# siyi-wind/MDViT

Hardware: AMD Instinct MI355X
Metric: 512x512 images/sec MDViT train step (fwd+bwd, two-sweep, AdamW) (higher is better)
Workload: dtype bf16x3 (fp32 storage; GEMM operands split hi+lo bf16, fp32 accumulate); 1 GPU; MDViT Sup+MLPFM train step, 4 domain(s) x bs=4 per GPU, 512x512, drop_rate=0.1 drop_path=0.1, bf16x3 GEMMs, data-parallel x1

## Files before the change

### include/mdvit_hip.h

```cpp
#ifndef MDVIT_HIP_H
#define MDVIT_HIP_H

#include <stddef.h>
#include <stdint.h>

#ifdef __cplusplus
extern "C" {
#endif

#define MDVIT_ABI_VERSION 1

enum {
    MDVIT_OK = 0,
    MDVIT_E_SHAPE = 1,
    MDVIT_E_DTYPE = 2,
    MDVIT_E_ALIGN = 3,
    MDVIT_E_WORKSPACE = 4,
    MDVIT_E_HIP = 5
};

enum { MDVIT_EPI_NONE = 0, MDVIT_EPI_GELU_DUAL = 1, MDVIT_EPI_DGELU = 2 };
enum { MDVIT_ACT_NONE = 0, MDVIT_ACT_HSWISH = 1, MDVIT_ACT_RELU = 2 };

const char* mdvit_last_error(void);
// ... 124 lines not shown
int mdvit_mlp_rc_bwd(const float* gm, const float* x, const void* W1p, const float* b1, const void* W2tp, const void* W1tp, float* dx_parts, float* dW1, float* db1,
                     float* dW2, void* ws, size_t ws_bytes, int32_t M, int32_t C, int32_t hidden, float drop_p, uint32_t key1_0, uint32_t key1_1,
                     const uint32_t* drop_seed, int32_t accumulate, void* stream);
size_t mdvit_mlp_rc_wgrad_ws_bytes(int32_t M, int32_t C, int32_t hidden);
int mdvit_mlp_rc_dgrad_masked(const float* g, const float* x, const void* W1p, const float* b1, const void* W2tp, const void* W1tp, float* dx, int32_t M, int32_t C,
                              int32_t hidden, float drop_p, uint32_t key1_0, uint32_t key1_1, const uint32_t* drop_seed, float mask_drop_p, uint32_t mask_key0,
                              uint32_t mask_key1, const uint32_t* mask_seed, const float* rowscale, int32_t rows_per_scale, void* stream);
int mdvit_mlp_rc16_dgrad_masked(const float* g, const float* x, const void* W1p, const float* b1, const void* W2tp, const void* W1tp, float* du, float* dx, float* gm_out,
                                int32_t M, int32_t C, int32_t hidden, float drop_p, uint32_t key1_0, uint32_t key1_1, const uint32_t* drop_seed, float mask_drop_p,
                                uint32_t mask_key0, uint32_t mask_key1, const uint32_t* mask_seed, const float* rowscale, int32_t rows_per_scale, void* stream);
int mdvit_mlp_rc16_dgrad_masked_hbf16(const float* g, const float* x, const void* W1p, const float* b1, const void* W2tp, const void* W1tp, float* du, float* dx,
                                      float* gm_out, int32_t M, int32_t C, int32_t hidden, float drop_p, uint32_t key1_0, uint32_t key1_1, const uint32_t* drop_seed,
                                      float mask_drop_p, uint32_t mask_key0, uint32_t mask_key1, const uint32_t* mask_seed, const float* rowscale,
                                      int32_t rows_per_scale, void* stream);
int mdvit_mlp_rc_wgrad_masked(const float* g, const float* x, const void* W1p, const float* b1, const void* W2tp, float* dW1, float* db1, float* dW2, void* ws,
                              size_t ws_bytes, int32_t M, int32_t C, int32_t hidden, float drop_p, uint32_t key1_0, uint32_t key1_1, const uint32_t* drop_seed,
                              float mask_drop_p, uint32_t mask_key0, uint32_t mask_key1, const uint32_t* mask_seed, const float* rowscale, int32_t rows_per_scale,
                              int32_t accumulate, void* stream);
int mdvit_mlp_rc_bwd_masked(const float* g, const float* x, const void* W1p, const float* b1, const void* W2tp, const void* W1tp, float* dx_parts, float* dW1, float* db1,
                            float* dW2, void* ws, size_t ws_bytes, int32_t M, int32_t C, int32_t hidden, float drop_p, uint32_t key1_0, uint32_t key1_1,
                            const uint32_t* drop_seed, float mask_drop_p, uint32_t mask_key0, uint32_t mask_key1, const uint32_t* mask_seed, const float* rowscale,
                            int32_t rows_per_scale, int32_t accumulate, void* stream);
int mdvit_mlp_mask_config(int32_t fold);
int mdvit_gemm_ledger(int32_t enable);
int mdvit_gemm_ledger_read(int32_t index, char* name, int32_t cap, int64_t* launches, double* flop, double* bytes);
int mdvit_gemm_sampler(const char* symbol, int32_t stride);
int mdvit_gemm_sampler_read(int32_t index, char* name, int32_t cap, int64_t* seen, int64_t* timed, double* ms);
int mdvit_mlp_rc_config(int32_t fwd_variant);
int mdvit_mlp_rc_planes(int32_t planes);
int mdvit_block_config(int32_t mlp_bwd_fused);
int mdvit_mlp_rc_wgrad(const float* gm, const float* x, const void* W1p, const float* b1, const void* W2tp, float* dW1, float* db1, float* dW2,
                       void* ws, size_t ws_bytes, int32_t M, int32_t C, int32_t hidden, float drop_p, uint32_t key1_0, uint32_t key1_1,
                       const uint32_t* drop_seed, int32_t accumulate, void* stream);

typedef struct MdvitBlockDesc {
    int32_t B, H, W, C, heads, hidden, s3, s5, s7, ln_groups, D, da_hidden, precision;
    float eps, drop_p;
    uint32_t key_proj[2], key_fc1[2], key_fc2[2];
    const uint32_t* drop_seed;
    const float* rowscale1; const float* rowscale2;
    const float* label;
    const float *cpe_w, *cpe_b, *n1_g, *n1_b, *qkv_w, *qkv_b, *w3, *b3, *w5, *b5, *w7, *b7, *da_w1, *da_b1, *da_w2, *da_b2, *proj_w, *proj_b, *n2_g, *n2_b, *fc1_w, *fc1_b,
        *fc2_w, *fc2_b;
    const float *qkv_wt, *proj_wt, *fc1_wt, *fc2_wt;
    const void *fc1_p, *fc2_p, *fc2t_p, *fc1t_p;
    const void *qkv_p, *proj_p, *projt_p, *qkvt_p;
// ... 252 lines not shown
```

### mdvit_amd/_lib.py

```python
from __future__ import annotations

import ctypes as C
import os
import re
from typing import List

_HERE = os.path.dirname(os.path.abspath(__file__))
LIB_PATH = os.environ.get("MDVIT_HIP_LIB") or os.path.join(_HERE, "lib", "libmdvit_hip.so")
HEADER_PATH = os.path.join(_HERE, "..", "include", "mdvit_hip.h")

EPI_NONE, EPI_GELU_DUAL, EPI_DGELU = 0, 1, 2
ACT_NONE, ACT_HSWISH, ACT_RELU = 0, 1, 2

f32p = C.c_void_p
vp = C.c_void_p
i32 = C.c_int32
i64 = C.c_int64
u32 = C.c_uint32
f32 = C.c_float


class GemmDesc(C.Structure):
    _fields_ = [
        ("A", vp), ("B", vp), ("C", vp), ("C2", vp),
# ... 107 lines not shown
    "mdvit_block_config": [i32],
    "mdvit_gemm_ledger": [i32],
    "mdvit_gemm_ledger_read": [i32, C.c_char_p, i32, C.POINTER(i64), C.POINTER(C.c_double), C.POINTER(C.c_double)],
    "mdvit_gemm_sampler": [C.c_char_p, i32],
    "mdvit_gemm_sampler_read": [i32, C.c_char_p, i32, C.POINTER(i64), C.POINTER(i64), C.POINTER(C.c_double)],
    "mdvit_mlp_rc_fwd": [vp, vp, vp, vp, vp, vp, vp, i32, vp, i32, i32, i32, f32, u32, u32, u32, u32, vp, vp],
    "mdvit_linear_rc": [vp, i64, vp, i64, vp, vp, i64, i32, i32, i32, f32, u32, u32, vp, i32, vp, i64, vp, vp],
    "mdvit_linear_rc_ln": [vp, vp, vp, i32, f32, vp, vp, vp, vp, i64, vp, vp, i64, i32, i32, i32, vp],
    "mdvit_mlp_rc_fwd_ln": [vp, vp, vp, i32, f32, vp, vp, vp, vp, vp, vp, vp, vp, i32, vp, vp, i32, i32, i32, f32, u32, u32, u32, u32, vp, vp],
    "mdvit_mlp_rc16_fwd": [vp, vp, vp, vp, vp, vp, vp, i32, vp, vp, i32, i32, i32, f32, u32, u32, u32, u32, vp, vp],
    "mdvit_mlp_rc_dgrad": [vp, vp, vp, vp, vp, vp, vp, i32, i32, i32, f32, u32, u32, vp, vp],
    "mdvit_mlp_rc16_dgrad": [vp, vp, vp, vp, vp, vp, vp, vp, i32, i32, i32, f32, u32, u32, vp, vp],
    "mdvit_mlp_rc_fwd_ln_hbf16": [vp, vp, vp, i32, f32, vp, vp, vp, vp, vp, vp, vp, vp, i32, vp, vp, i32, i32, i32, f32, u32, u32, u32, u32, vp, vp],
    "mdvit_mlp_rc16_fwd_hbf16": [vp, vp, vp, vp, vp, vp, vp, i32, vp, vp, i32, i32, i32, f32, u32, u32, u32, u32, vp, vp],
    "mdvit_mlp_rc16_dgrad_hbf16": [vp, vp, vp, vp, vp, vp, vp, vp, i32, i32, i32, f32, u32, u32, vp, vp],
    "mdvit_mlp_rc_wgrad": [vp, vp, vp, vp, vp, vp, vp, vp, vp, C.c_size_t, i32, i32, i32, f32, u32, u32, vp, i32, vp],
    "mdvit_mlp_rc_bwd": [vp, vp, vp, vp, vp, vp, vp, vp, vp, vp, vp, C.c_size_t, i32, i32, i32, f32, u32, u32, vp, i32, vp],
    "mdvit_mlp_rc_dgrad_masked": [vp, vp, vp, vp, vp, vp, vp, i32, i32, i32, f32, u32, u32, vp, f32, u32, u32, vp, vp, i32, vp],
    "mdvit_mlp_rc16_dgrad_masked": [vp, vp, vp, vp, vp, vp, vp, vp, vp, i32, i32, i32, f32, u32, u32, vp, f32, u32, u32, vp, vp, i32, vp],
    "mdvit_mlp_rc16_dgrad_masked_hbf16": [vp, vp, vp, vp, vp, vp, vp, vp, vp, i32, i32, i32, f32, u32, u32, vp, f32, u32, u32, vp, vp, i32, vp],
    "mdvit_mlp_rc_wgrad_masked": [vp, vp, vp, vp, vp, vp, vp, vp, vp, C.c_size_t, i32, i32, i32, f32, u32, u32, vp, f32, u32, u32, vp, vp, i32, i32, vp],
    "mdvit_mlp_rc_bwd_masked": [vp, vp, vp, vp, vp, vp, vp, vp, vp, vp, vp, C.c_size_t, i32, i32, i32, f32, u32, u32, vp, f32, u32, u32, vp, vp, i32, i32, vp],
    "mdvit_mlp_mask_config": [i32],
    "mdvit_imgconv_fwd": [vp, vp, vp, i32, i32, i32, i32, i32, i32, vp],
    "mdvit_imgconv_wgrad": [vp, vp, vp, vp, C.c_size_t, i32, i32, i32, i32, i32, i32, i32, vp],
    "mdvit_maxpool3x3s2_fwd": [vp, vp, vp, i32, i32, i32, i32, vp],
    "mdvit_maxpool3x3s2_bwd": [vp, vp, vp, i32, i32, i32, i32, vp],
    "mdvit_resize_ac_fwd": [vp, vp, i32, i32, i32, i32, i32, i32, vp],
    "mdvit_resize_ac_bwd": [vp, vp, i32, i32, i32, i32, i32, i32, vp],
    "mdvit_ew": [vp, vp, vp, i64, i32, vp],
    "mdvit_add3": [vp, vp, vp, vp, i64, vp],
    "mdvit_add_parts": [vp, vp, C.POINTER(vp), i32, i64, vp, vp],
    "mdvit_add_bcast": [vp, vp, vp, i32, i64, vp],
    "mdvit_sum_batch": [vp, vp, i32, i64, vp],
    "mdvit_gate_fwd": [vp, vp, vp, i32, i64, i32, i32, vp],
    "mdvit_gate_bwd": [vp, vp, vp, vp, vp, vp, C.c_size_t, i32, i64, i32, i32, vp],
    "mdvit_imgconv_im2col": [vp, vp, i32, i32, i32, i32, i32, i32, vp],
    "mdvit_chanpool_fwd": [vp, vp, vp, i64, i32, vp],
    "mdvit_chanpool_bwd": [vp, vp, vp, i64, i32, vp],
    "mdvit_conv7x7_2to1_fwd": [vp, vp, vp, i32, i32, i32, vp],
    "mdvit_conv7x7_2to1_bwd": [vp, vp, vp, vp, vp, i32, i32, i32, vp],
    "mdvit_bn1_fwd": [vp, vp, vp, vp, vp, vp, vp, vp, i64, i32, i32, f32, f32, vp],
    "mdvit_bn1_bwd": [vp, vp, vp, vp, vp, vp, i64, i32, i32, vp],
    "mdvit_subsample2": [vp, vp, i32, i32, i32, i32, i32, vp],
    "mdvit_patchify": [vp, vp, i32, i32, i32, i32, i32, vp],
    "mdvit_dropout2d": [vp, vp, i32, i64, i32, f32, u32, u32, vp, vp],
# ... 204 lines not shown
```

### mdvit_amd/csrc/mlp_rc.hip

```cpp
#include "common.h"
#include <type_traits>
#ifndef RC_ABL
#define RC_ABL 0
#endif

typedef float rc_f32x16 __attribute__((ext_vector_type(16)));
typedef __bf16 rc_bf16x8 __attribute__((ext_vector_type(8)));
typedef unsigned rc_u4 __attribute__((ext_vector_type(4)));
typedef unsigned rc_u2 __attribute__((ext_vector_type(2)));
typedef float rc_f4 __attribute__((ext_vector_type(4)));
typedef short rc_v4i16 __attribute__((ext_vector_type(4)));
typedef short rc_v8i16 __attribute__((ext_vector_type(8)));
typedef __attribute__((address_space(3))) rc_v4i16* rc_lds_v4i16_ptr;

namespace {

template <int ROWB>
__device__ __forceinline__ int rc_swz(int row) {
    if (ROWB == 64) return (row >> 2) & 3;
    if (ROWB == 128) return (((row >> 1) & 1) << 2) | ((row >> 2) & 3);
    return row & 15;
}

template <int ROWB>
__device__ __forceinline__ void rc_glds_piece(const uint16_t* __restrict__ src, long ld, int piece, int lane, char* tile) {
    constexpr int LPR = ROWB / 16, RPP = 1024 / ROWB;
    const int row = piece * RPP + lane / LPR;
    const int lc = (lane % LPR) ^ rc_swz<ROWB>(row);
    __builtin_amdgcn_global_load_lds(src + (long)row * ld + (lc << 3), (__attribute__((address_space(3))) void*)(tile + piece * 1024), 16, 0, 0);
}

template <int ROWB>
__device__ __forceinline__ rc_bf16x8 rc_frag(const char* tile, int row, int chunk) {
    return __builtin_bit_cast(rc_bf16x8, *reinterpret_cast<const rc_u4*>(tile + row * ROWB + ((chunk ^ rc_swz<ROWB>(row)) << 4)));
}

// ... 183 lines not shown
            *reinterpret_cast<float4*>(ln.out + (long)row * K + 8 * lhi + 16 * kb + 4) = b[kb];
        }
    }
    if (lhi == 0 && row < M) { ln.mean[row] = mu; ln.rstd[row] = rs; }
}

struct RcArgs {
    const float* x; const float* gm; const float* res; const float* rowscale; const float* b1; const float* b2;
    const uint16_t* W1p;
    const uint16_t* W2p;
    const uint16_t* W2tp;
    const uint16_t* W1tp;
    float* y; float* dx;
    float* du;
    int hbf;
    float* h;
    LnPro ln;
    RcMask mk;
    float* part;
    int M, Hd, rows_per_scale;
    int drop; uint32_t k1a, k1b, k2a, k2b, thresh; float inv_keep;
    const uint32_t* seed;
    int groups, tiles_per_group;
};

template <int NM, int V, int ND, int LEAD>
__device__ __forceinline__ void rc_interleave() {
    __builtin_amdgcn_sched_group_barrier(0x100, LEAD, 0);
#pragma unroll
    for (int i = 0; i < NM; ++i) {
        __builtin_amdgcn_sched_group_barrier(0x008, 1, 0);
        __builtin_amdgcn_sched_group_barrier(0x002, V, 0);
        if (i < ND - LEAD) __builtin_amdgcn_sched_group_barrier(0x100, 1, 0);
    }
}

#define RC_WAIT_VM(n) asm volatile("s_waitcnt vmcnt(%0)" ::"n"(n) : "memory")
#define RC_BARRIER() asm volatile("s_waitcnt lgkmcnt(0)\n\ts_barrier" ::: "memory")

template <int C, int NW, bool DROP>
__global__ __launch_bounds__(NW * 64) __attribute__((amdgpu_waves_per_eu(2, 2))) void mlp_rc_fwd_kernel(RcArgs p) {
    constexpr int KB = C / 16, CB = C / 32;
    constexpr int RB1 = C * 2;
    constexpr int T1 = 32 * RB1, T2 = C * 64;
    constexpr int PIECES = (2 * T1 + 2 * T2) / 1024;
    static_assert(PIECES % NW == 0, "pieces must divide over the waves");
    constexpr int PPW = PIECES / NW;
// ... 149 lines not shown
}


template <int C, int NW, bool DROP, int OCC = 3, bool STORE = false, bool LNP = false, bool P1 = false>
__global__ __launch_bounds__(NW * 64) __attribute__((amdgpu_waves_per_eu(OCC, OCC))) void mlp_rc_fwd3_kernel(RcArgs p) {
    constexpr int KB = C / 16, CB = C / 32;
    constexpr int RB1 = C * 2;
    constexpr int T1 = 32 * RB1, T2 = C * 64;
    static_assert(T1 == T2 && T1 / 1024 == NW, "one 1 KiB piece of each of the four planes (W1 hi, lo, W2 hi, lo) per wave and hidden step");
    constexpr int PPW = 4;
    extern __shared__ __attribute__((aligned(1024))) char smem[];
    char* sW1 = smem;
    char* sW2 = sW1 + 3 * 2 * T1;
    float* sB1 = reinterpret_cast<float*>(sW2 + 3 * 2 * T2);
    const int tid = threadIdx.x, lane = tid & 63, wave = __builtin_amdgcn_readfirstlane(tid >> 6), l31 = lane & 31, lhi = lane >> 5;
    const int row = blockIdx.x * (NW * 32) + wave * 32 + l31;
    const int n = p.Hd >> 5;
    uint32_t s0 = 0, s1 = 0;
    if (p.seed) { s0 = p.seed[0]; s1 = p.seed[1]; }
    const uint32_t k1a = p.k1a ^ s0, k1b = p.k1b + s1, k2a = p.k2a ^ s0, k2b = p.k2b + s1;
    const uint32_t dq0 = (uint32_t)((long)row * p.Hd + 4 * lhi) >> 2, thresh16 = p.thresh >> 16;
    const float hki = 0.5f * p.inv_keep;
    const long wplane = (long)p.Hd * C;
    uint32_t voff1, voff2;
    {
        constexpr int LPR = RB1 / 16, RPP = 1024 / RB1;
        const int r1 = wave * RPP + lane / LPR;
        voff1 = (uint32_t)(r1 * C + (((lane % LPR) ^ rc_swz<RB1>(r1)) << 3)) * 2u;
        const int r2 = wave * 16 + (lane >> 2);
        voff2 = (uint32_t)(r2 * p.Hd + (((lane & 3) ^ rc_swz<64>(r2)) << 3)) * 2u;
    }
    const char* gW1 = reinterpret_cast<const char*>(p.W1p);
    const char* gW2 = reinterpret_cast<const char*>(p.W2p);
    auto issue_group = [&](int g, int slot) __attribute__((always_inline)) {
        const int gs = min(g, n - 1);
        const char* b1p = gW1 + (long)gs * (32 * C * 2);
        const char* b2p = gW2 + (long)gs * (32 * 2);
        typedef __attribute__((address_space(3))) void* lds_ptr;
        __builtin_amdgcn_global_load_lds(b1p + voff1, (lds_ptr)(sW1 + (slot * 2 + 0) * T1 + wave * 1024), 16, 0, 0);
        __builtin_amdgcn_global_load_lds(b1p + wplane * 2 + voff1, (lds_ptr)(sW1 + (slot * 2 + 1) * T1 + wave * 1024), 16, 0, 0);
        __builtin_amdgcn_global_load_lds(b2p + voff2, (lds_ptr)(sW2 + (slot * 2 + 0) * T2 + wave * 1024), 16, 0, 0);
        __builtin_amdgcn_global_load_lds(b2p + wplane * 2 + voff2, (lds_ptr)(sW2 + (slot * 2 + 1) * T2 + wave * 1024), 16, 0, 0);
    };
    issue_group(0, 0);
    issue_group(1, 1);
    for (int i = tid; i < p.Hd / 4; i += NW * 64) reinterpret_cast<float4*>(sB1)[i] = reinterpret_cast<const float4*>(p.b1)[i];
// ... 101 lines not shown

template <int C, int NW, bool DROP, bool P1 = false>
__global__ __launch_bounds__(NW * 64) __attribute__((amdgpu_waves_per_eu(2, 2))) void mlp_rc_dgrad_kernel(RcArgs p) {
    constexpr int KB = C / 16, CB = C / 32;
    constexpr int RB1 = C * 2;
    constexpr int T1 = 32 * RB1, T3 = C * 64;
    constexpr int PIECES = (4 * T1 + 2 * T3) / 1024;
    static_assert(PIECES % NW == 0, "pieces must divide over the waves");
    constexpr int PPW = PIECES / NW;
    extern __shared__ __attribute__((aligned(1024))) char smem[];
    char* sW1 = smem;
    char* sW2t = sW1 + 3 * 2 * T1;
    char* sW1t = sW2t + 3 * 2 * T1;
    float* sB1 = reinterpret_cast<float*>(sW1t + 3 * 2 * T3);
    const int tid = threadIdx.x, lane = tid & 63, wave = __builtin_amdgcn_readfirstlane(tid >> 6), l31 = lane & 31, lhi = lane >> 5;
    const int row = blockIdx.x * (NW * 32) + wave * 32 + l31;
    const int n = p.Hd >> 5;
    uint32_t s0 = 0, s1 = 0;
    if (p.seed) { s0 = p.seed[0]; s1 = p.seed[1]; }
    const uint32_t k1a = p.k1a ^ s0, k1b = p.k1b + s1;
    const uint32_t dq0 = (uint32_t)((long)row * p.Hd + 4 * lhi) >> 2, thresh16 = p.thresh >> 16;
    const float hks = 0.5f * p.inv_keep, pks = 0.39894228040143268f * p.inv_keep;
    const long wplane = (long)p.Hd * C;

    static_assert(T1 / 1024 == NW && T3 / 1024 == NW, "one 1 KiB piece of each of the six planes per wave and hidden step");
    uint32_t voff1, voff3;
    {
        constexpr int LPR = RB1 / 16, RPP = 1024 / RB1;
        const int r1 = wave * RPP + lane / LPR;
        voff1 = (uint32_t)(r1 * C + (((lane % LPR) ^ rc_swz<RB1>(r1)) << 3)) * 2u;
        const int r3 = wave * 16 + (lane >> 2);
        voff3 = (uint32_t)(r3 * p.Hd + (((lane & 3) ^ rc_swz<64>(r3)) << 3)) * 2u;
    }
    typedef __attribute__((address_space(3))) void* lds_ptr;
    auto issue_a = [&](int slot_s, int src_s) __attribute__((always_inline)) {
        const int sl = slot_s % 3;
        const char* b1p = reinterpret_cast<const char*>(p.W1p) + (long)src_s * (32 * C * 2);
        const char* b2p = reinterpret_cast<const char*>(p.W2tp) + (long)src_s * (32 * C * 2);
        __builtin_amdgcn_global_load_lds(b1p + voff1, (lds_ptr)(sW1 + (sl * 2 + 0) * T1 + wave * 1024), 16, 0, 0);
        __builtin_amdgcn_global_load_lds(b1p + wplane * 2 + voff1, (lds_ptr)(sW1 + (sl * 2 + 1) * T1 + wave * 1024), 16, 0, 0);
        __builtin_amdgcn_global_load_lds(b2p + voff1, (lds_ptr)(sW2t + (sl * 2 + 0) * T1 + wave * 1024), 16, 0, 0);
        __builtin_amdgcn_global_load_lds(b2p + wplane * 2 + voff1, (lds_ptr)(sW2t + (sl * 2 + 1) * T1 + wave * 1024), 16, 0, 0);
    };
    auto issue_b = [&](int s) __attribute__((always_inline)) {
        const int sl = s % 3;
        const char* b3p = reinterpret_cast<const char*>(p.W1tp) + (long)s * (32 * 2);
// ... 226 lines not shown
            }
        }
        if (row >= p.M) rg = make_float4(0.f, 0.f, 0.f, 0.f);
    };
    auto store_tile = [&](int buf, int t) __attribute__((always_inline)) {
        char* b = smem + buf * 4 * TP;
        uint2 hi, lo;
        mdvit_split_bf16x3(rx, hi, lo);
        *reinterpret_cast<rc_u2*>(b + soff) = rc_u2{hi.x, hi.y};
        *reinterpret_cast<rc_u2*>(b + TP + soff) = rc_u2{lo.x, lo.y};
        if (p.mk.on) rg = rc_mask4(rg, rsc, p.mk.drop != 0, mk0, mk1, (uint32_t)((long)min(t * 32 + srow, p.M - 1) * C + sc4 * 4), p.mk.thresh, p.mk.inv_keep);
        mdvit_split_bf16x3(rg, hi, lo);
        *reinterpret_cast<rc_u2*>(b + 2 * TP + soff) = rc_u2{hi.x, hi.y};
        *reinterpret_cast<rc_u2*>(b + 3 * TP + soff) = rc_u2{lo.x, lo.y};
    };

    if (DX) {
        for (int i = tid; i < 2 * 64 * 32; i += 512) {
            const int pl = i >> 11, c = (i >> 5) & 63, ch = i & 31;
            const rc_u4 v = *reinterpret_cast<const rc_u4*>(p.W1tp + pl * wplane + (long)c * p.Hd + role * 256 + ch * 8);
            *reinterpret_cast<rc_u4*>(sWt + (pl * 64 + c) * RC_WT_ROW + ch * 16) = v;
        }
    }
    if (t_beg < t_end) {
        load_tile(t_beg);
        store_tile(0, t_beg);
    }
    __syncthreads();
    for (int t = t_beg; t < t_end; ++t) {
        const int buf = (t - t_beg) & 1;
        const char* xb = smem + buf * 4 * TP;
        const char* xhi = xb; const char* xlo = xb + TP; const char* ghi = xb + 2 * TP; const char* glo = xb + 3 * TP;
        if (t + 1 < t_end) load_tile(t + 1);
        rc_f32x16 u, d;
#pragma unroll
        for (int r = 0; r < 16; ++r) { u[r] = bias; d[r] = 0.f; }
#pragma unroll
        for (int kb = 0; kb < KB; ++kb) {
            const rc_bf16x8 ah = rc_frag<128>(xhi, l31, 2 * kb + lhi), al = rc_frag<128>(xlo, l31, 2 * kb + lhi);
            RC_MFMA3_ACT_AP(P1, u, ah, al, w1h[kb], w1l[kb]);
            const rc_bf16x8 ch = rc_frag<128>(ghi, l31, 2 * kb + lhi), cl = rc_frag<128>(glo, l31, 2 * kb + lhi);
            RC_MFMA3_ACT_AP(P1, d, ch, cl, w2h[kb], w2l[kb]);
        }
        uint32_t hb[4];
        if (DROP) {
#pragma unroll
            for (int j = 0; j < 4; ++j) {
                const int tok = t * 32 + j + 8 * (lane & 3) + 4 * lhi;
                hb[j] = mdvit_drop_bits(k1a, k1b, (uint32_t)((long)tok * p.Hd + hs + l31));
            }
        }
#pragma unroll
        for (int ks = 0; ks < 2; ++ks) {
            rc_u4 hh, hl, dh, dl;
#pragma unroll
            for (int i = 0; i < 4; ++i) {
// ... 39 lines not shown
        }
        if (DX) {
            __syncthreads();
            const int cblk = wave & 3, tblk = wave >> 2, g4 = lane >> 4;
            rc_acc4 acc = {0.f, 0.f, 0.f, 0.f};
            const int pr = l15 >> 2, pcb = 32 * tblk + 8 * (l15 & 3);
#pragma unroll
            for (int k8 = 0; k8 < 8; ++k8) {
                const char* wa = sWt + (cblk * 16 + l15) * RC_WT_ROW + (4 * k8 + g4) * 16;
                const rc_bf16x8 ah = __builtin_bit_cast(rc_bf16x8, *reinterpret_cast<const rc_u4*>(wa));
                const rc_bf16x8 al = __builtin_bit_cast(rc_bf16x8, *reinterpret_cast<const rc_u4*>(wa + 64 * RC_WT_ROW));
                const char* dplane = sDu + k8 * 4096;
                const int ra = 8 * g4 + pr, rb = ra + 4;
                const int oa = ra * 64 + (((pcb >> 4) ^ ((ra >> 1) & 3)) << 4) + (pcb & 15), ob = rb * 64 + (((pcb >> 4) ^ ((rb >> 1) & 3)) << 4) + (pcb & 15);
                const rc_v4i16 h0 = __builtin_amdgcn_ds_read_tr16_b64_v4i16((rc_lds_v4i16_ptr)(dplane + oa)), h1 = __builtin_amdgcn_ds_read_tr16_b64_v4i16((rc_lds_v4i16_ptr)(dplane + ob));
                const rc_v4i16 l0 = __builtin_amdgcn_ds_read_tr16_b64_v4i16((rc_lds_v4i16_ptr)(dplane + 2048 + oa)), l1 = __builtin_amdgcn_ds_read_tr16_b64_v4i16((rc_lds_v4i16_ptr)(dplane + 2048 + ob));
                const rc_bf16x8 bh = __builtin_bit_cast(rc_bf16x8, (rc_v8i16{h0[0], h0[1], h0[2], h0[3], h1[0], h1[1], h1[2], h1[3]}));
                const rc_bf16x8 bl = __builtin_bit_cast(rc_bf16x8, (rc_v8i16{l0[0], l0[1], l0[2], l0[3], l1[0], l1[1], l1[2], l1[3]}));
                RC16_MFMA3_BWDP(P1, acc, ah, al, bh, bl);
            }
            const int tok = t * 32 + tblk * 16 + l15;
            if (tok < p.M) *reinterpret_cast<float4*>(p.dx + ((long)role * p.M + tok) * C + cblk * 16 + 4 * g4) = make_float4(acc[0], acc[1], acc[2], acc[3]);
        }
        if (t + 1 < t_end) store_tile(buf ^ 1, t + 1);
        __syncthreads();
    }

    float* pg = p.part + (long)group * (2L * p.Hd * C + p.Hd);
#pragma unroll
    for (int cb = 0; cb < CB; ++cb)
#pragma unroll
        for (int r = 0; r < 16; ++r) {
            const int i = (r & 3) + 8 * (r >> 2) + 4 * lhi;
            pg[(long)(hs + i) * C + cb * 32 + l31] = aw1[cb][r];
            pg[(long)p.Hd * C + (long)(cb * 32 + i) * p.Hd + hs + l31] = aw2[cb][r];
        }
    db1 += __shfl_xor(db1, 32, 64);
    if (lhi == 0) pg[2L * p.Hd * C + hs + l31] = db1;
}

typedef float rc_f32x4 __attribute__((ext_vector_type(4)));

template <int ROWB>
__device__ __forceinline__ int rc16_swz(int row) {
    if (ROWB == 64) return (row >> 2) & 3;
    if (ROWB == 128) return (row >> 1) & 7;
    return row & 15;
// ... 119 lines not shown
}

template <int C, int NW, int OCC, bool DROP, bool STORE, bool LNP = false, bool P1 = false>
__global__ __launch_bounds__(NW * 64) __attribute__((amdgpu_waves_per_eu(OCC, OCC))) void mlp_rc16_fwd_kernel(RcArgs p) {
    constexpr int KS = C / 32, CT = C / 16;
    constexpr int RB1 = C * 2;
    constexpr int T1 = 32 * RB1, T2 = C * 64;
    constexpr int PIECES = (2 * T1 + 2 * T2) / 1024;
    static_assert(PIECES % NW == 0, "pieces must divide over the waves");
    constexpr int PPW = PIECES / NW;
    extern __shared__ __attribute__((aligned(1024))) char smem[];
    char* sW1 = smem;
    char* sW2 = sW1 + 3 * 2 * T1;
    float* sB1 = reinterpret_cast<float*>(sW2 + 3 * 2 * T2);
    const int tid = threadIdx.x, lane = tid & 63, wave = __builtin_amdgcn_readfirstlane(tid >> 6), c16 = lane & 15, g = lane >> 4;
    const int row = blockIdx.x * (NW * 16) + wave * 16 + c16;
    const int n = p.Hd >> 5;
    uint32_t s0 = 0, s1 = 0;
    if (p.seed) { s0 = p.seed[0]; s1 = p.seed[1]; }
    const uint32_t k1a = p.k1a ^ s0, k1b = p.k1b + s1, k2a = p.k2a ^ s0, k2b = p.k2b + s1;
    const uint32_t dq0 = (uint32_t)((long)row * p.Hd + 4 * g) >> 2, thresh16 = p.thresh >> 16;
    const float hki = 0.5f * p.inv_keep;
    const long wplane = (long)p.Hd * C;
    auto issue_group = [&](int gi) __attribute__((always_inline)) {
        const int gs = min(gi, n - 1), slot = gi % 3;
#pragma unroll
        for (int i = 0; i < PPW; ++i) {
            const int pc = wave + i * NW;
            if (pc < 2 * T1 / 1024) {
                constexpr int PP = T1 / 1024;
                const int pl = pc / PP, q = pc % PP;
                rc16_glds_piece<RB1>(p.W1p + pl * wplane + (long)(gs * 32) * C, C, q, lane, sW1 + (slot * 2 + pl) * T1);
            } else {
                constexpr int PP = T2 / 1024;
                const int pc2 = pc - 2 * T1 / 1024, pl = pc2 / PP, q = pc2 % PP;
                rc16_glds_piece<64>(p.W2p + pl * wplane + gs * 32, p.Hd, q, lane, sW2 + (slot * 2 + pl) * T2);
            }
        }
    };
    issue_group(0);
    issue_group(1);
    for (int i = tid; i < p.Hd / 4; i += NW * 64) reinterpret_cast<float4*>(sB1)[i] = reinterpret_cast<const float4*>(p.b1)[i];
    rc_bf16x8 xh[KS], xl[KS];
    rc16_load_rows<C, LNP>(p.x, row, p.M, g, xh, xl, &p.ln);
    rc_f32x4 yacc[CT];
#pragma unroll
// ... 71 lines not shown

template <int C, int NW, int OCC, bool DROP, bool STORE, bool P1 = false>
__global__ __launch_bounds__(NW * 64) __attribute__((amdgpu_waves_per_eu(OCC, OCC))) void mlp_rc16_dgrad_kernel(RcArgs p) {
    constexpr int KS = C / 32, CT = C / 16;
    constexpr int RB1 = C * 2;
    constexpr int T1 = 32 * RB1, T3 = C * 64;
    constexpr int PIECES = (4 * T1 + 2 * T3) / 1024;
    static_assert(PIECES % NW == 0, "pieces must divide over the waves");
    constexpr int PPW = PIECES / NW;
    extern __shared__ __attribute__((aligned(1024))) char smem[];
    char* sW1 = smem;
    char* sW2 = sW1 + 3 * 2 * T1;
    char* sW3 = sW2 + 3 * 2 * T1;
    float* sB1 = reinterpret_cast<float*>(sW3 + 3 * 2 * T3);
    const int tid = threadIdx.x, lane = tid & 63, wave = __builtin_amdgcn_readfirstlane(tid >> 6), c16 = lane & 15, g = lane >> 4;
    const int row = blockIdx.x * (NW * 16) + wave * 16 + c16;
    const int n = p.Hd >> 5;
    uint32_t s0 = 0, s1 = 0;
    if (p.seed) { s0 = p.seed[0]; s1 = p.seed[1]; }
    const uint32_t k1a = p.k1a ^ s0, k1b = p.k1b + s1;
    const uint32_t dq0 = (uint32_t)((long)row * p.Hd + 4 * g) >> 2, thresh16 = p.thresh >> 16;
    const float hks = 0.5f * p.inv_keep, pks = 0.39894228040143268f * p.inv_keep;
    const long wplane = (long)p.Hd * C;
    auto issue_group = [&](int gi) __attribute__((always_inline)) {
        const int gs = min(gi, n - 1), slot = gi % 3;
#pragma unroll
        for (int i = 0; i < PPW; ++i) {
            const int pc = wave + i * NW;
            constexpr int PP1 = T1 / 1024, PP3 = T3 / 1024;
            if (pc < 2 * PP1) {
                const int pl = pc / PP1, q = pc % PP1;
                rc16_glds_piece<RB1>(p.W1p + pl * wplane + (long)(gs * 32) * C, C, q, lane, sW1 + (slot * 2 + pl) * T1);
            } else if (pc < 4 * PP1) {
                const int pc2 = pc - 2 * PP1, pl = pc2 / PP1, q = pc2 % PP1;
                rc16_glds_piece<RB1>(p.W2tp + pl * wplane + (long)(gs * 32) * C, C, q, lane, sW2 + (slot * 2 + pl) * T1);
            } else {
                const int pc3 = pc - 4 * PP1, pl = pc3 / PP3, q = pc3 % PP3;
                rc16_glds_piece<64>(p.W1tp + pl * wplane + gs * 32, p.Hd, q, lane, sW3 + (slot * 2 + pl) * T3);
            }
        }
    };
    issue_group(0);
    issue_group(1);
    for (int i = tid; i < p.Hd / 4; i += NW * 64) reinterpret_cast<float4*>(sB1)[i] = reinterpret_cast<const float4*>(p.b1)[i];
    rc_bf16x8 xh[KS], xl[KS], mh[KS], ml[KS];
    rc16_load_rows<C>(p.x, row, p.M, g, xh, xl);
// ... 182 lines not shown
    }
    const int i = q * 4;
    float* dst = i < n0 ? o0 + i : (i < n0 + n1 ? o1 + (i - n0) : o2 + (i - n0 - n1));
    float4 v = s;
    if (accumulate) { const float4 o = *reinterpret_cast<const float4*>(dst); v.x += o.x; v.y += o.y; v.z += o.z; v.w += o.w; }
    *reinterpret_cast<float4*>(dst) = v;
}

int rc_set_lds(const void* k, int bytes, bool (&flags)[64]) {
    int dev = 0;
    if (hipGetDevice(&dev) != hipSuccess || dev < 0 || dev >= 64) dev = 0;
    if (flags[dev]) return MDVIT_OK;
    const hipError_t e = hipFuncSetAttribute(k, hipFuncAttributeMaxDynamicSharedMemorySize, bytes);
    if (e != hipSuccess) return mdvit_set_error(MDVIT_E_HIP, "mlp_rc: cannot raise the dynamic LDS limit: %s", hipGetErrorString(e));
    flags[dev] = true;
    return MDVIT_OK;
}

void rc_fill(RcArgs& a, int M, int Hd, float drop_p, uint32_t k10, uint32_t k11, uint32_t k20, uint32_t k21, const uint32_t* seed) {
    a.M = M; a.Hd = Hd;
    a.drop = drop_p > 0.f; a.k1a = k10; a.k1b = k11; a.k2a = k20; a.k2b = k21;
    a.thresh = mdvit_drop_thresh(drop_p); a.inv_keep = 1.f / (1.f - drop_p);
    a.seed = seed;
}

int rc_mask_fill(RcMask& m, const char* who, int M, int C, float drop_p, uint32_t key0, uint32_t key1, const uint32_t* seed, const float* rowscale, int rows_per_scale,
                 float* gm_out) {
    MDVIT_CHECK_ARG(drop_p >= 0.f && drop_p < 1.f, MDVIT_E_SHAPE, "%s: mask drop_p must lie in [0, 1)", who);
    MDVIT_CHECK_ARG(!(drop_p > 0.f) || (long)M * C < (1L << 32), MDVIT_E_SHAPE, "%s: mask index space exceeds 2^32", who);
    MDVIT_CHECK_ARG(aligned16(gm_out), MDVIT_E_ALIGN, "%s: gm_out must be 16-byte aligned", who);
    memset(&m, 0, sizeof(m));
    m.on = drop_p > 0.f || rowscale != nullptr;
    if (!m.on) return MDVIT_OK;
    m.drop = drop_p > 0.f; m.k0 = key0; m.k1 = key1; m.seed = m.drop ? seed : nullptr;
    m.thresh = mdvit_drop_thresh(drop_p); m.inv_keep = 1.f / (1.f - drop_p);
    m.rowscale = rowscale; m.rows_per_scale = rows_per_scale > 0 ? rows_per_scale : 1; m.gm_out = gm_out;
    return MDVIT_OK;
}

}

int g_rc_planes = 2;
extern "C" int mdvit_mlp_rc_planes(int32_t planes) {
    if (planes != 1 && planes != 2) return mdvit_set_error(MDVIT_E_SHAPE, "mlp_rc_planes: 1 or 2");
    g_rc_planes = planes;
    return MDVIT_OK;
// ... 461 lines not shown
    return MDVIT_OK;
}

extern "C" int mdvit_mlp_rc_bwd(const float* gm, const float* x, const void* W1p, const float* b1, const void* W2tp, const void* W1tp, float* dx_parts,
                                float* dW1, float* db1, float* dW2, void* ws, size_t ws_bytes, int32_t M, int32_t C, int32_t Hd, float drop_p,
                                uint32_t key1_0, uint32_t key1_1, const uint32_t* drop_seed, int32_t accumulate, void* stream) {
    return rc_bwd_impl(nullptr, gm, x, W1p, b1, W2tp, W1tp, dx_parts, dW1, db1, dW2, ws, ws_bytes, M, C, Hd, drop_p, key1_0, key1_1, drop_seed, accumulate, stream);
}
extern "C" int mdvit_mlp_rc_bwd_masked(const float* g, const float* x, const void* W1p, const float* b1, const void* W2tp, const void* W1tp, float* dx_parts,
                                       float* dW1, float* db1, float* dW2, void* ws, size_t ws_bytes, int32_t M, int32_t C, int32_t Hd, float drop_p,
                                       uint32_t key1_0, uint32_t key1_1, const uint32_t* drop_seed, float mask_drop_p, uint32_t mask_key0, uint32_t mask_key1,
                                       const uint32_t* mask_seed, const float* rowscale, int32_t rows_per_scale, int32_t accumulate, void* stream) {
    RcMask mk;
    const int rc = rc_mask_fill(mk, "mlp_rc_bwd_masked", M, C, mask_drop_p, mask_key0, mask_key1, mask_seed, rowscale, rows_per_scale, nullptr);
    if (rc != MDVIT_OK) return rc;
    return rc_bwd_impl(&mk, g, x, W1p, b1, W2tp, W1tp, dx_parts, dW1, db1, dW2, ws, ws_bytes, M, C, Hd, drop_p, key1_0, key1_1, drop_seed, accumulate, stream);
}

int g_rc_mask_fold = MDVIT_MASK_FOLD_DEFAULT;
extern "C" int mdvit_mlp_mask_config(int32_t fold) {
    g_rc_mask_fold = fold == 1 ? MDVIT_MASK_FOLD_DEFAULT : (fold & (MDVIT_MASK_FOLD_AUX | MDVIT_MASK_FOLD_FULL128 | MDVIT_MASK_FOLD_FULL64));
    return MDVIT_OK;
}
```

### mdvit_amd/ops.py

```python
from __future__ import annotations

import ctypes as C
import itertools
import os
import weakref
from typing import Optional, Tuple

import torch

from . import _lib
from ._lib import GemmDesc, call

_key_counter = itertools.count(1)
_POISON = os.environ.get("MDVIT_POISON", "0") == "1"


def _empty(*a, **k):
    t = torch.empty(*a, **k)
    if _POISON and t.is_floating_point():
        t.fill_(float("nan"))
    return t


def _empty_like(x):
# ... 1099 lines not shown

_mlp_recompute = os.environ.get("MDVIT_MLP_RECOMPUTE", "1") != "0"
_mlp_fused = os.environ.get("MDVIT_MLP_FUSED", "1") != "0"
_mlp_recompute_maxc = int(os.environ.get("MDVIT_MLP_RECOMPUTE_MAXC", "128"))
_mlp_rc = os.environ.get("MDVIT_MLP_RC", "1") != "0"
_mlp_rc16 = os.environ.get("MDVIT_MLP_RC16", "1") != "0"
_mlp_rc_bwd = os.environ.get("MDVIT_MLP_RC_BWD", "1")
_lib.on_load(lambda lib: lib.mdvit_block_config({"0": 0, "1": 1}.get(_mlp_rc_bwd, 2)))
_MASK_FOLD_AUX, _MASK_FOLD_FULL128, _MASK_FOLD_FULL64 = 2, 4, 8
_MASK_FOLD_DEFAULT = _MASK_FOLD_AUX | _MASK_FOLD_FULL128 | _MASK_FOLD_FULL64
_mlp_mask_fold = _MASK_FOLD_DEFAULT


def set_mlp_mask_fold(v: int) -> None:
    global _mlp_mask_fold
    v = int(v)
    _mlp_mask_fold = _MASK_FOLD_DEFAULT if v == 1 else v & (_MASK_FOLD_AUX | _MASK_FOLD_FULL128 | _MASK_FOLD_FULL64)
    _lib.on_load(lambda lib, v=v: lib.mdvit_mlp_mask_config(v))


_mlp_mask_fold_env = os.environ.get("MDVIT_MLP_MASK_FOLD", "1")
if _mlp_mask_fold_env != "1":
    set_mlp_mask_fold(int(_mlp_mask_fold_env))


def _mlp_rc_ok(Cin, Hd, b1, b2, res, W1, W2, M) -> bool:
    return (_mlp_rc and _mlp_recompute and _gemm_precision >= 1 and Cin == 64 and Hd % 256 == 0 and Hd <= 4096 and b1 is not None and b2 is not None and res is not None
            and W1.is_contiguous() and W2.is_contiguous() and M * Hd < (1 << 32))


def _mlp_rc16_ok(Cin, Hd, b1, W1, W2, M) -> bool:
    return (_mlp_rc16 and _gemm_precision >= 1 and Cin == 128 and Hd % 32 == 0 and Hd <= 4096 and b1 is not None and W1.is_contiguous() and W2.is_contiguous()
            and M * Hd < (1 << 32))


class _MlpResidual(torch.autograd.Function):
    @staticmethod
    def forward(ctx, x, res, W1, b1, W2, b2, rowscale, drop_p, rows_per_scale):
        ctx.set_materialize_grads(False)
        _chk(x, res, W1, b1, W2, b2, rowscale)
        M, Cin = x.shape
        Hd = W1.shape[0]
        k1 = _next_key() if drop_p > 0 else (0, 0)
        k2 = _next_key() if drop_p > 0 else (0, 0)
        if _mlp_rc_ok(Cin, Hd, b1, b2, res, W1, W2, M):
            out = _empty((M, Cin), device=x.device, dtype=torch.float32)
# ... 2229 lines not shown
```

Baseline: 546.2 images/s.

## Skip MLP fwd/bwd work for rows zeroed by drop-path rowscale

Adds a drop-path skip path to the recompute MLP kernels. When every row in a block has a zero rowscale (the sample was dropped by drop_path), the forward copies the residual to the output and zeroes the hidden store, and the backward writes zero dx/gm/du. The wgrad kernel steps its tile loop past dead row runs. This avoids GEMM work on samples whose MLP branch contributes nothing, at the cost of extra rowscale reads and branching, with gains depending on how many samples the random drop-path removes.

```diff
diff --git a/include/mdvit_hip.h b/include/mdvit_hip.h
--- a/include/mdvit_hip.h
+++ b/include/mdvit_hip.h
@@ -170,6 +170,7 @@
                             const uint32_t* drop_seed, float mask_drop_p, uint32_t mask_key0, uint32_t mask_key1, const uint32_t* mask_seed, const float* rowscale,
                             int32_t rows_per_scale, int32_t accumulate, void* stream);
 int mdvit_mlp_mask_config(int32_t fold);
+int mdvit_droppath_skip_config(int32_t skip);
 int mdvit_gemm_ledger(int32_t enable);
 int mdvit_gemm_ledger_read(int32_t index, char* name, int32_t cap, int64_t* launches, double* flop, double* bytes);
 int mdvit_gemm_sampler(const char* symbol, int32_t stride);
diff --git a/mdvit_amd/_lib.py b/mdvit_amd/_lib.py
--- a/mdvit_amd/_lib.py
+++ b/mdvit_amd/_lib.py
@@ -153,6 +153,7 @@
     "mdvit_mlp_rc_wgrad_masked": [vp, vp, vp, vp, vp, vp, vp, vp, vp, C.c_size_t, i32, i32, i32, f32, u32, u32, vp, f32, u32, u32, vp, vp, i32, i32, vp],
     "mdvit_mlp_rc_bwd_masked": [vp, vp, vp, vp, vp, vp, vp, vp, vp, vp, vp, C.c_size_t, i32, i32, i32, f32, u32, u32, vp, f32, u32, u32, vp, vp, i32, i32, vp],
     "mdvit_mlp_mask_config": [i32],
+    "mdvit_droppath_skip_config": [i32],
     "mdvit_imgconv_fwd": [vp, vp, vp, i32, i32, i32, i32, i32, i32, vp],
     "mdvit_imgconv_wgrad": [vp, vp, vp, vp, C.c_size_t, i32, i32, i32, i32, i32, i32, i32, vp],
     "mdvit_maxpool3x3s2_fwd": [vp, vp, vp, i32, i32, i32, i32, vp],
diff --git a/mdvit_amd/csrc/mlp_rc.hip b/mdvit_amd/csrc/mlp_rc.hip
--- a/mdvit_amd/csrc/mlp_rc.hip
+++ b/mdvit_amd/csrc/mlp_rc.hip
@@ -12,6 +12,8 @@
 typedef short rc_v4i16 __attribute__((ext_vector_type(4)));
 typedef short rc_v8i16 __attribute__((ext_vector_type(8)));
 typedef __attribute__((address_space(3))) rc_v4i16* rc_lds_v4i16_ptr;
+
+int g_rc_droppath_skip = 1;
 
 namespace {
 
@@ -241,7 +243,20 @@
     int drop; uint32_t k1a, k1b, k2a, k2b, thresh; float inv_keep;
     const uint32_t* seed;
     int groups, tiles_per_group;
+    int skip;
 };
+
+__device__ __forceinline__ bool rc_rows_dead(const float* __restrict__ rowscale, int rows_per_scale, int r0, int r1) {
+    if (!rowscale) return false;
+    bool dead = true;
+    for (int q = r0 / rows_per_scale, q1 = r1 / rows_per_scale; dead && q <= q1; ++q) dead = rowscale[q] == 0.0f;
+    return dead;
+}
+__device__ __forceinline__ void rc_zero_hidden_row(float* base, long row, int Hd, int hbf, int l, int nl) {
+    const int rowb = Hd * (hbf ? 2 : 4);
+    uint4* dst = reinterpret_cast<uint4*>(reinterpret_cast<char*>(base) + row * rowb);
+    for (int i = l; i < (rowb >> 4); i += nl) dst[i] = make_uint4(0u, 0u, 0u, 0u);
+}
 
 template <int NM, int V, int ND, int LEAD>
 __device__ __forceinline__ void rc_interleave() {
@@ -437,6 +452,26 @@
     const uint32_t dq0 = (uint32_t)((long)row * p.Hd + 4 * lhi) >> 2, thresh16 = p.thresh >> 16;
     const float hki = 0.5f * p.inv_keep;
     const long wplane = (long)p.Hd * C;
+    if (p.skip) {
+        const int r0 = blockIdx.x * (NW * 32);
+        if (rc_rows_dead(p.rowscale, p.rows_per_scale, r0, min(r0 + NW * 32, p.M) - 1)) {
+            if constexpr (LNP) {
+                rc_bf16x8 xh[KB], xl[KB];
+                rc_load_rows<C, true>(p.x, row, p.M, lhi, xh, xl, &p.ln);
+            }
+            if (row < p.M) {
+#pragma unroll
+                for (int cb = 0; cb < CB; ++cb)
+#pragma unroll
+                    for (int q = 0; q < 4; ++q) {
+                        const long o = (long)row * C + cb * 32 + 8 * q + 4 * lhi;
+                        *reinterpret_cast<float4*>(p.y + o) = *reinterpret_cast<const float4*>(p.res + o);
+                    }
+                if (STORE) rc_zero_hidden_row(p.h, row, p.Hd, 0, lhi, 2);
+            }
+            return;
+        }
+    }
     uint32_t voff1, voff2;
     {
         constexpr int LPR = RB1 / 16, RPP = 1024 / RB1;
@@ -584,6 +619,19 @@
     const uint32_t dq0 = (uint32_t)((long)row * p.Hd + 4 * lhi) >> 2, thresh16 = p.thresh >> 16;
     const float hks = 0.5f * p.inv_keep, pks = 0.39894228040143268f * p.inv_keep;
     const long wplane = (long)p.Hd * C;
+    if (p.skip && p.mk.on) {
+        const int r0 = blockIdx.x * (NW * 32);
+        if (rc_rows_dead(p.mk.rowscale, p.mk.rows_per_scale, r0, min(r0 + NW * 32, p.M) - 1)) {
+            if (row < p.M) {
+#pragma unroll
+                for (int cb = 0; cb < CB; ++cb)
+#pragma unroll
+                    for (int q = 0; q < 4; ++q)
+                        *reinterpret_cast<float4*>(p.dx + (long)row * C + cb * 32 + 8 * q + 4 * lhi) = make_float4(0.f, 0.f, 0.f, 0.f);
+            }
+            return;
+        }
+    }
 
     static_assert(T1 / 1024 == NW && T3 / 1024 == NW, "one 1 KiB piece of each of the six planes per wave and hidden step");
     uint32_t voff1, voff3;
@@ -856,16 +904,49 @@
             *reinterpret_cast<rc_u4*>(sWt + (pl * 64 + c) * RC_WT_ROW + ch * 16) = v;
         }
     }
-    if (t_beg < t_end) {
-        load_tile(t_beg);
-        store_tile(0, t_beg);
+    const bool skipping = p.skip && p.mk.on && p.mk.rowscale;
+    auto classify = [&](int t, int& run_end) __attribute__((always_inline)) {
+        const int r0 = t * 32, r1 = min(r0 + 32, p.M) - 1, q1 = r1 / p.mk.rows_per_scale;
+        const bool dead = rc_rows_dead(p.mk.rowscale, p.mk.rows_per_scale, r0, r1);
+        const long e = ((long)q1 + 1) * p.mk.rows_per_scale;
+        long u = t + 1;
+        if (dead) u = e / 32;
+        else if (p.mk.rowscale[q1] != 0.0f) u = (e - 1) / 32 + 1;
+        run_end = __builtin_amdgcn_readfirstlane((int)min(max(u, (long)t + 1), (long)t_end));
+        return dead;
+    };
+    int live_until = skipping ? t_beg : t_end;
+    auto next_live = [&](int t) __attribute__((always_inline)) {
+        while (t < t_end && t >= live_until) {
+            int e;
+            if (classify(t, e)) t = e;
+            else live_until = e;
+        }
+        return __builtin_amdgcn_readfirstlane(t);
+    };
+    if (DX && skipping) {
+        for (int t = t_beg; t < t_end;) {
+            int e;
+            if (classify(t, e)) {
+                for (int tt = t; tt < e; ++tt) {
+                    const int row = tt * 32 + srow;
+                    if (row < p.M) *reinterpret_cast<float4*>(p.dx + ((long)role * p.M + row) * C + sc4 * 4) = make_float4(0.f, 0.f, 0.f, 0.f);
+                }
+            }
+            t = e;
+        }
+    }
+    const int t_first = next_live(t_beg);
+    if (t_first < t_end) {
+        load_tile(t_first);
+        store_tile(0, t_first);
     }
     __syncthreads();
-    for (int t = t_beg; t < t_end; ++t) {
-        const int buf = (t - t_beg) & 1;
+    for (int t = t_first, buf = 0, t_next; t < t_end; t = t_next, buf ^= 1) {
+        t_next = next_live(t + 1);
         const char* xb = smem + buf * 4 * TP;
         const char* xhi = xb; const char* xlo = xb + TP; const char* ghi = xb + 2 * TP; const char* glo = xb + 3 * TP;
-        if (t + 1 < t_end) load_tile(t + 1);
+        if (t_next < t_end) load_tile(t_next);
         rc_f32x16 u, d;
 #pragma unroll
         for (int r = 0; r < 16; ++r) { u[r] = bias; d[r] = 0.f; }
@@ -951,7 +1032,7 @@
             const int tok = t * 32 + tblk * 16 + l15;
             if (tok < p.M) *reinterpret_cast<float4*>(p.dx + ((long)role * p.M + tok) * C + cblk * 16 + 4 * g4) = make_float4(acc[0], acc[1], acc[2], acc[3]);
         }
-        if (t + 1 < t_end) store_tile(buf ^ 1, t + 1);
+        if (t_next < t_end) store_tile(buf ^ 1, t_next);
         __syncthreads();
     }
 
@@ -1117,6 +1198,24 @@
     const uint32_t dq0 = (uint32_t)((long)row * p.Hd + 4 * g) >> 2, thresh16 = p.thresh >> 16;
     const float hki = 0.5f * p.inv_keep;
     const long wplane = (long)p.Hd * C;
+    if (p.skip) {
+        const int r0 = blockIdx.x * (NW * 16);
+        if (rc_rows_dead(p.rowscale, p.rows_per_scale, r0, min(r0 + NW * 16, p.M) - 1)) {
+            if constexpr (LNP) {
+                rc_bf16x8 xh[KS], xl[KS];
+                rc16_load_rows<C, true>(p.x, row, p.M, g, xh, xl, &p.ln);
+            }
+            if (row < p.M) {
+#pragma unroll
+                for (int ct = 0; ct < CT; ++ct) {
+                    const long o = (long)row * C + 16 * ct + 4 * g;
+                    *reinterpret_cast<float4*>(p.y + o) = *reinterpret_cast<const float4*>(p.res + o);
+                }
+                if (STORE) rc_zero_hidden_row(p.h, row, p.Hd, p.hbf, g, 4);
+            }
+            return;
+        }
+    }
     auto issue_group = [&](int gi) __attribute__((always_inline)) {
         const int gs = min(gi, n - 1), slot = gi % 3;
 #pragma unroll
@@ -1234,6 +1333,21 @@
     const uint32_t dq0 = (uint32_t)((long)row * p.Hd + 4 * g) >> 2, thresh16 = p.thresh >> 16;
     const float hks = 0.5f * p.inv_keep, pks = 0.39894228040143268f * p.inv_keep;
     const long wplane = (long)p.Hd * C;
+    if (p.skip && p.mk.on) {
+        const int r0 = blockIdx.x * (NW * 16);
+        if (rc_rows_dead(p.mk.rowscale, p.mk.rows_per_scale, r0, min(r0 + NW * 16, p.M) - 1)) {
+            if (row < p.M) {
+#pragma unroll
+                for (int ct = 0; ct < CT; ++ct) {
+                    const long o = (long)row * C + 16 * ct + 4 * g;
+                    *reinterpret_cast<float4*>(p.dx + o) = make_float4(0.f, 0.f, 0.f, 0.f);
+                    if (p.mk.gm_out) *reinterpret_cast<float4*>(p.mk.gm_out + o) = make_float4(0.f, 0.f, 0.f, 0.f);
+                }
+                if (STORE) rc_zero_hidden_row(p.du, row, p.Hd, p.hbf, g, 4);
+            }
+            return;
+        }
+    }
     auto issue_group = [&](int gi) __attribute__((always_inline)) {
         const int gs = min(gi, n - 1), slot = gi % 3;
 #pragma unroll
@@ -1462,6 +1576,7 @@
     a.drop = drop_p > 0.f; a.k1a = k10; a.k1b = k11; a.k2a = k20; a.k2b = k21;
     a.thresh = mdvit_drop_thresh(drop_p); a.inv_keep = 1.f / (1.f - drop_p);
     a.seed = seed;
+    a.skip = g_rc_droppath_skip;
 }
 
 int rc_mask_fill(RcMask& m, const char* who, int M, int C, float drop_p, uint32_t key0, uint32_t key1, const uint32_t* seed, const float* rowscale, int rows_per_scale,
@@ -1969,3 +2084,8 @@
     g_rc_mask_fold = fold == 1 ? MDVIT_MASK_FOLD_DEFAULT : (fold & (MDVIT_MASK_FOLD_AUX | MDVIT_MASK_FOLD_FULL128 | MDVIT_MASK_FOLD_FULL64));
     return MDVIT_OK;
 }
+
+extern "C" int mdvit_droppath_skip_config(int32_t skip) {
+    g_rc_droppath_skip = skip != 0;
+    return MDVIT_OK;
+}
diff --git a/mdvit_amd/ops.py b/mdvit_amd/ops.py
--- a/mdvit_amd/ops.py
+++ b/mdvit_amd/ops.py
@@ -1145,6 +1145,15 @@
 _mlp_mask_fold_env = os.environ.get("MDVIT_MLP_MASK_FOLD", "1")
 if _mlp_mask_fold_env != "1":
     set_mlp_mask_fold(int(_mlp_mask_fold_env))
+
+
+def set_droppath_skip(v: int) -> None:
+    _lib.on_load(lambda lib, v=int(v): lib.mdvit_droppath_skip_config(v))
+
+
+_droppath_skip_env = os.environ.get("MDVIT_DROPPATH_SKIP", "1")
+if _droppath_skip_env != "1":
+    set_droppath_skip(int(_droppath_skip_env))
 
 
 def _mlp_rc_ok(Cin, Hd, b1, b2, res, W1, W2, M) -> bool:
```

Result: no change. 548.2 images/s (median of 6 runs) (+0.4%).
